# ortk95/planetmapper

Hardware: NVIDIA B200
Metric: full-backplane Mpix/s (FP64) + mapped-cube voxels/s at 1-8 B200 vs host CPU (higher is better)
Workload: dtype f64

## Files before the change

planetmapper_b200/csrc/backplane_kernels.cu:

```cuda
#include "pm_device.cuh"
#include "pm_kernels.h"

#include <cstdlib>

namespace pm {

constexpr int kPerThread = 4;
#ifndef PM_IMG_PARAM_CTAS
#define PM_IMG_PARAM_CTAS 4
#endif
constexpr int kImgParamCtas = PM_IMG_PARAM_CTAS;

__device__ __forceinline__ int slot(uint64_t mask, int k) { return __popcll(mask & (bit(k) - 1ull)); }

struct PlaneOffsets {
    int64_t byte_off[PM_N_PLANES];
    int64_t frame_stride;
};
static PlaneOffsets make_plane_offsets(uint64_t mask, int64_t plane_stride) {
    PlaneOffsets po;
    int slot = 0;
    for (int k = 0; k < PM_N_PLANES; k++) {
        po.byte_off[k] = (int64_t)slot * plane_stride * (int64_t)sizeof(double);
        if (mask & bit(k)) slot++;
    }
    po.frame_stride = (int64_t)slot * plane_stride;
    return po;
}

struct PlaneSink {
    char *base;
    const PlaneOffsets &po;
    __device__ __forceinline__ void put(int k, double v) const {
        __stcs(reinterpret_cast<double *>(base + po.byte_off[k]), v);
    }
};

template <bool kSky, uint64_t kFixedMask, bool kSpinSym>
__device__ __forceinline__ void img_tile(const FrameD &fs, uint32_t tile, uint32_t nx, uint32_t npx, int per_thread,
                                         uint64_t mask, const PlaneOffsets &po, double *__restrict__ out) {
    uint32_t idx = tile * (uint32_t)(kBlock * per_thread) + threadIdx.x;
    uint32_t yi = idx / nx, xi = idx - yi * nx;
#pragma unroll 1
    for (int r = 0; r < per_thread && idx < npx; r++) {
        PlaneSink sink{reinterpret_cast<char *>(out + idx), po};
        image_pixel<kSky, kFixedMask, false, kSpinSym>(fs, (double)xi, (double)yi, mask, sink);
        idx += kBlock;
        xi += kBlock;
        while (xi >= nx) {
            xi -= nx;
            yi++;
        }
    }
}

template <bool kSky, uint64_t kFixedMask>
__global__ void __launch_bounds__(kBlock, 4) backplanes_img_kernel(const PMFrame *__restrict__ frames, uint32_t nx,
                                                                   uint32_t npx, int per_thread, uint64_t mask,
                                                                   const __grid_constant__ PlaneOffsets po,
                                                                   double *__restrict__ out_all) {
    __shared__ FrameD fs;
    load_frame(fs, frames + blockIdx.y);
    double *out = out_all + (int64_t)blockIdx.y * __popcll(mask) * npx;
    if (fs.spin_sym)
        img_tile<kSky, kFixedMask, true>(fs, blockIdx.x, nx, npx, per_thread, mask, po, out);
    else
        img_tile<kSky, kFixedMask, false>(fs, blockIdx.x, nx, npx, per_thread, mask, po, out);
}

__device__ __forceinline__ uint32_t centre_out_tile(uint32_t k, uint32_t n_tiles, uint32_t centre) {
    const uint32_t lo = centre, hi = n_tiles - 1u - centre;
    const uint32_t j = (k + 1u) >> 1;
    if (j <= min(lo, hi)) return (k & 1u) ? centre + j : centre - j;
    return lo < hi ? k : n_tiles - 1u - k;
}
template <bool kSky, uint64_t kFixedMask, bool kSpinSym>
__global__ void __launch_bounds__(kBlock, kImgParamCtas) backplanes_img_param_kernel(
    const __grid_constant__ FrameD fs, uint32_t nx, uint32_t npx, int per_thread, uint32_t centre_tile, uint64_t mask,
    const __grid_constant__ PlaneOffsets po, double *__restrict__ out) {
    img_tile<kSky, kFixedMask, kSpinSym>(fs, centre_out_tile(blockIdx.x, gridDim.x, centre_tile), nx, npx, per_thread,
                                         mask, po, out);
}

template <bool kSky, bool kRingAll, bool kSpinSym>
__global__ void __launch_bounds__(kBlock, 4) backplanes_points_param_kernel(const __grid_constant__ FrameD fs,
                                                                            const double *__restrict__ x_in,
                                                                            const double *__restrict__ y_in,
                                                                            int64_t n, uint64_t mask,
                                                                            const __grid_constant__ PlaneOffsets po,
                                                                            double *__restrict__ out) {
    const int64_t first = (int64_t)blockIdx.x * (kBlock * kPerThread) + threadIdx.x;
#pragma unroll 1
    for (int r = 0; r < kPerThread; r++) {
        const int64_t idx = first + r * kBlock;
        if (idx >= n) break;
        PlaneSink sink{reinterpret_cast<char *>(out + idx), po};
        image_point<kSky, kRingAll, kSpinSym>(fs, __ldg(x_in + idx), __ldg(y_in + idx), mask, sink);
    }
}

constexpr uint64_t kXYMapMask = bit(PM_PIXEL_X) | bit(PM_PIXEL_Y);

template <uint64_t kFixedMask>
__device__ __forceinline__ void map_tile(const FrameD &fs, const double *__restrict__ lon_in,
                                         const double *__restrict__ lat_in, int64_t n, uint64_t mask,
                                         const PlaneOffsets &po, double *__restrict__ out) {
    const int64_t first = (int64_t)blockIdx.x * (kBlock * kPerThread) + threadIdx.x;
#pragma unroll 1
    for (int r = 0; r < kPerThread; r++) {
        const int64_t idx = first + r * kBlock;
        if (idx >= n) break;
        PlaneSink sink{reinterpret_cast<char *>(out + idx), po};
        map_cell<kFixedMask>(fs, __ldg(lon_in + idx), __ldg(lat_in + idx), mask, sink);
    }
// ... 198 lines not shown
                                  int64_t n, double *__restrict__ out) {
    const int64_t i = (int64_t)blockIdx.x * blockDim.x + threadIdx.x;
    if (i >= n) return;
    const double x = a[i], y = b ? b[i] : 0.0;
    double s, c, r = NAN;
    switch (kind) {
        case 0: r = fast_rcp(x); break;
        case 1: r = fast_rsqrt(x); break;
        case 2: r = fast_sqrt(x); break;
        case 3: sincos_small(x, s, c); r = s; break;
        case 4: sincos_small(x, s, c); r = c; break;
        case 5: r = fast_atan2(x, y); break;
        case 6: r = fast_acos(x); break;
        case 7: r = fast_div(x, y); break;
        case 8: sincos_full(x, s, c); r = s; break;
        case 9: sincos_full(x, s, c); r = c; break;
        case 10: r = fast_atan2_ypos(fabs(x), y); break;
        case 11: r = fast_atan2_xpos(x, fabs(y)); break;
        case 12: sincos_small2(x, 0.0, s, c, r, r); r = s; break;
        case 13: sincos_small2(x, 0.0, s, c, r, r); r = c; break;
        default: break;
    }
    out[i] = r;
}

static unsigned chunks_for(int64_t n) {
    const int64_t per = (int64_t)kBlock * kPerThread;
    int64_t blocks = (n + per - 1) / per;
    return (unsigned)(blocks < 1 ? 1 : blocks);
}

constexpr uint64_t kDefaultStackMask = kLonLatMask | kCentricMask | kIllumMask | kStateMask;

static int pick_per_thread(int64_t n, int64_t n_batches, int sm_count, int ctas_per_sm) {
    const int64_t tiles = ((n + kBlock - 1) / kBlock) * n_batches;
    const int64_t target = (int64_t)sm_count * ctas_per_sm * 3;
    int per = 16;
    while (per > 1 && tiles / per < target) per >>= 1;
    return per;
}

cudaError_t launch_backplanes_img(const PMFrame *frames, int n_frames, int nx, int ny, uint64_t mask,
                                  double *out, int sm_count, cudaStream_t st) {
    const int64_t npx = (int64_t)nx * ny;
    if (npx >= (1ll << 31)) return cudaErrorInvalidValue;
    const PlaneOffsets po = make_plane_offsets(mask, npx);
    static const int forced = tune_int("PM_IMG_PER_THREAD", 0);
    const int per = forced > 0 ? forced : pick_per_thread(npx, n_frames, sm_count, 4);
    const int64_t chunk = (int64_t)kBlock * per;
    dim3 grid((unsigned)((npx + chunk - 1) / chunk), n_frames);
    static const bool no_fixed = tune_int("PM_IMG_NO_FIXED_MASK", 0) != 0;
    if (mask == kDefaultStackMask && !no_fixed)
        backplanes_img_kernel<false, kDefaultStackMask><<<grid, kBlock, 0, st>>>(frames, (uint32_t)nx, (uint32_t)npx,
                                                                                   per, mask, po, out);
    else if (mask & kSkyMask)
        backplanes_img_kernel<true, 0><<<grid, kBlock, 0, st>>>(frames, (uint32_t)nx, (uint32_t)npx, per, mask, po, out);
    else
        backplanes_img_kernel<false, 0><<<grid, kBlock, 0, st>>>(frames, (uint32_t)nx, (uint32_t)npx, per, mask, po, out);
    count_launches(1);
    return cudaGetLastError();
}
template <bool kSpinSym>
static void launch_img_param(const FrameD &fs, dim3 grid, uint32_t nx, uint32_t npx, int per, uint32_t centre,
                             uint64_t mask, const PlaneOffsets &po, double *out, cudaStream_t st) {
    if (mask == kDefaultStackMask)
        backplanes_img_param_kernel<false, kDefaultStackMask, kSpinSym><<<grid, kBlock, 0, st>>>(fs, nx, npx, per, centre,
                                                                                                mask, po, out);
    else if (mask & kSkyMask)
        backplanes_img_param_kernel<true, 0, kSpinSym><<<grid, kBlock, 0, st>>>(fs, nx, npx, per, centre, mask, po, out);
    else
        backplanes_img_param_kernel<false, 0, kSpinSym><<<grid, kBlock, 0, st>>>(fs, nx, npx, per, centre, mask, po, out);
}
cudaError_t launch_backplanes_img_host(const PMFrame *frame_host, int nx, int ny, uint64_t mask, double *out,
                                       int sm_count, cudaStream_t st) {
    const int64_t npx = (int64_t)nx * ny;
    if (npx >= (1ll << 31)) return cudaErrorInvalidValue;
    FrameD fs;
    load_frame_host(fs, frame_host);
    const PlaneOffsets po = make_plane_offsets(mask, npx);
    static const int forced = tune_int("PM_IMG_PER_THREAD", 0);
    const int per = forced > 0 ? forced : pick_per_thread(npx, 1, sm_count, kImgParamCtas);
    const int64_t chunk = (int64_t)kBlock * per;
    const int64_t n_tiles = (npx + chunk - 1) / chunk;
    dim3 grid((unsigned)n_tiles, 1);
    double cy = frame_host->y0 < 0.0 ? 0.0 : (frame_host->y0 > ny - 1.0 ? ny - 1.0 : frame_host->y0);
    double cx = frame_host->x0 < 0.0 ? 0.0 : (frame_host->x0 > nx - 1.0 ? nx - 1.0 : frame_host->x0);
    if (!(cy == cy) || !(cx == cx)) cy = cx = 0.0;
    int64_t ct = ((int64_t)cy * nx + (int64_t)cx) / chunk;
    static const bool linear = tune_int("PM_IMG_ORDER", 1) == 0;
    if (linear) ct = 0;
    const uint32_t centre = (uint32_t)(ct < 0 ? 0 : (ct >= n_tiles ? n_tiles - 1 : ct));
    if (fs.spin_sym)
        launch_img_param<true>(fs, grid, (uint32_t)nx, (uint32_t)npx, per, centre, mask, po, out, st);
    else
        launch_img_param<false>(fs, grid, (uint32_t)nx, (uint32_t)npx, per, centre, mask, po, out, st);
    count_launches(1);
    return cudaGetLastError();
}
template <bool kSpinSym>
static void launch_points_param(const FrameD &fs, unsigned grid, const double *x, const double *y, int64_t n,
                                uint64_t mask, uint32_t flags, const PlaneOffsets &po, double *out, cudaStream_t st) {
    if (!(mask & kSkyMask))
        backplanes_points_param_kernel<false, false, kSpinSym><<<grid, kBlock, 0, st>>>(fs, x, y, n, mask, po, out);
    else if (flags & PM_FLAG_RING_ALL)
        backplanes_points_param_kernel<true, true, kSpinSym><<<grid, kBlock, 0, st>>>(fs, x, y, n, mask, po, out);
    else
        backplanes_points_param_kernel<true, false, kSpinSym><<<grid, kBlock, 0, st>>>(fs, x, y, n, mask, po, out);
}
cudaError_t launch_backplanes_points_host(const PMFrame *frame_host, const double *x, const double *y, int64_t n,
                                          uint64_t mask, uint32_t flags, double *out, cudaStream_t st) {
    FrameD fs;
    load_frame_host(fs, frame_host);
    const PlaneOffsets po = make_plane_offsets(mask, n);
    const unsigned grid = chunks_for(n);
    if (fs.spin_sym)
        launch_points_param<true>(fs, grid, x, y, n, mask, flags, po, out, st);
    else
        launch_points_param<false>(fs, grid, x, y, n, mask, flags, po, out, st);
    count_launches(1);
    return cudaGetLastError();
}
cudaError_t launch_backplanes_map(const PMFrame *frames, int n_frames, const double *lon, const double *lat,
                                  int64_t n, uint64_t mask, double *out, int sm_count, cudaStream_t st) {
    (void)sm_count;
    const dim3 grid(chunks_for(n), (unsigned)n_frames);
    const PlaneOffsets po = make_plane_offsets(mask, n);
    if (mask == kXYMapMask)
        backplanes_map_kernel<kXYMapMask><<<grid, kBlock, 0, st>>>(frames, lon, lat, n, mask, po, out);
// ... 87 lines not shown
```

planetmapper_b200/csrc/pm_device.cuh:

```cuda
#pragma once

#include "../../include/pm_b200.h"
#include "pm_math.cuh"

namespace pm {

struct V3 {
    double x, y, z;
};

PM_HD V3 mk(double x, double y, double z) { return V3{x, y, z}; }
PM_HD V3 operator+(V3 a, V3 b) { return mk(a.x + b.x, a.y + b.y, a.z + b.z); }
PM_HD V3 operator-(V3 a, V3 b) { return mk(a.x - b.x, a.y - b.y, a.z - b.z); }
PM_HD V3 operator-(V3 a) { return mk(-a.x, -a.y, -a.z); }
PM_HD V3 operator*(double s, V3 a) { return mk(s * a.x, s * a.y, s * a.z); }
PM_HD double dot(V3 a, V3 b) { return fma(a.x, b.x, fma(a.y, b.y, a.z * b.z)); }
PM_HD V3 cross(V3 a, V3 b) {
    return mk(fma(a.y, b.z, -a.z * b.y), fma(a.z, b.x, -a.x * b.z), fma(a.x, b.y, -a.y * b.x));
}
PM_HD V3 mul3(V3 a, const double *s) { return mk(a.x * s[0], a.y * s[1], a.z * s[2]); }
PM_HD V3 axpy(double s, V3 b, V3 a) { return mk(fma(s, b.x, a.x), fma(s, b.y, a.y), fma(s, b.z, a.z)); }
PM_HD double norm(V3 a) { return fast_sqrt_lite(dot(a, a)); }
PM_HD V3 ld3(const double *p) { return mk(p[0], p[1], p[2]); }
PM_HD bool finite3(V3 a) { return fabs(a.x) < INFINITY && fabs(a.y) < INFINITY && fabs(a.z) < INFINITY; }
PM_HD V3 mxv(const double *m, V3 v) {
    return mk(fma(m[0], v.x, fma(m[1], v.y, m[2] * v.z)), fma(m[3], v.x, fma(m[4], v.y, m[5] * v.z)),
              fma(m[6], v.x, fma(m[7], v.y, m[8] * v.z)));
}
PM_HD V3 mtxv(const double *m, V3 v) {
    return mk(fma(m[0], v.x, fma(m[3], v.y, m[6] * v.z)), fma(m[1], v.x, fma(m[4], v.y, m[7] * v.z)),
              fma(m[2], v.x, fma(m[5], v.y, m[8] * v.z)));
}
PM_HD_NOINLINE double pymod360_slow(double a) {
    double r = ::fmod(a, 360.0);
    if (r != 0.0 && r < 0.0) r += 360.0;
    return r;
}
PM_HD double pymod360(double a) { return (a >= 0.0 && a < 360.0) ? a : pymod360_slow(a); }

struct FrameD {
    PMFrame f;
    double inv_c;
    double inv_r[3];
    double nw[3];
    double k[3];
    double wn;
    double rp;
    double e2, ep2;
    double inv_omf2;
    double omf;
    double P0b[3], VTb[3], ATb[3], VOb[3], S0b[3], VSb[3];
    double G[9];
    double y0[3];
    double y0m2;
    double As[6];
    double inv_kmpa;
    int biaxial;
    int spin_sym;
};

constexpr int kDeriveItems = 13;

PM_HD double ex_mul(double a, double b) {
#ifdef __CUDA_ARCH__
    return __dmul_rn(a, b);
#else
    return a * b;
#endif
}
PM_HD double ex_add(double a, double b) {
#ifdef __CUDA_ARCH__
    return __dadd_rn(a, b);
#else
    return a + b;
#endif
}
PM_HD double ex_div(double a, double b) {
#ifdef __CUDA_ARCH__
    return __ddiv_rn(a, b);
#else
    return a / b;
#endif
}
PM_HD double ex_sqrt(double a) {
#ifdef __CUDA_ARCH__
    return __dsqrt_rn(a);
#else
    return ::sqrt(a);
#endif
}
PM_HD double ex_dot3(double a0, double b0, double a1, double b1, double a2, double b2) {
    return ex_add(ex_add(ex_mul(a0, b0), ex_mul(a1, b1)), ex_mul(a2, b2));
}

PM_HD void derive_frame_item(FrameD &s, int item) {
    const PMFrame &f = s.f;
    if (item >= 3 && item <= 8) {
        const double *src = item == 3 ? f.P0 : item == 4 ? f.VT : item == 5 ? f.AT : item == 6 ? f.VO : item == 7 ? f.S0 : f.VS;
        double *dst = item == 3 ? s.P0b : item == 4 ? s.VTb : item == 5 ? s.ATb : item == 6 ? s.VOb : item == 7 ? s.S0b : s.VSb;
        for (int r = 0; r < 3; r++)
            dst[r] = ex_dot3(f.R0[3 * r], src[0], f.R0[3 * r + 1], src[1], f.R0[3 * r + 2], src[2]);
        if (item == 3) {
            for (int r = 0; r < 3; r++) s.y0[r] = ex_mul(-dst[r], ex_div(1.0, f.radii[r]));
            s.y0m2 = fma(s.y0[0], s.y0[0], fma(s.y0[1], s.y0[1], ex_mul(s.y0[2], s.y0[2])));
        }
    } else if (item >= 9 && item <= 11) {
        const int r = item - 9;
        for (int c = 0; c < 3; c++)
            s.G[3 * r + c] = ex_dot3(f.R0[3 * r], f.M[3 * c], f.R0[3 * r + 1], f.M[3 * c + 1], f.R0[3 * r + 2], f.M[3 * c + 2]);
    } else if (item == 12) {
        const double sc = kRpd / 3600.0;
        for (int c = 0; c < 3; c++) {
            s.As[c] = -ex_mul(f.A[c], sc);
            s.As[3 + c] = ex_mul(f.A[3 + c], sc);
        }
        s.inv_kmpa = ex_div(1.0, f.km_per_arcsec);
    } else if (item == 0) {
        s.inv_c = ex_div(1.0, f.clight);
        const double w2 = ex_dot3(f.omega[0], f.omega[0], f.omega[1], f.omega[1], f.omega[2], f.omega[2]);
        const double wn = ex_sqrt(w2);
        s.wn = wn;
        s.k[0] = wn > 0.0 ? ex_div(f.omega[0], wn) : 0.0;
        s.k[1] = wn > 0.0 ? ex_div(f.omega[1], wn) : 0.0;
        s.k[2] = wn > 0.0 ? ex_div(f.omega[2], wn) : 0.0;
        const double wperp = ex_sqrt(ex_add(ex_mul(f.omega[0], f.omega[0]), ex_mul(f.omega[1], f.omega[1])));
        const double flat = fabs(ex_add(f.radii[0], -f.radii[2]));
        const double shift = ex_mul(ex_mul(wperp, ex_div(ex_mul(2.0, f.radii[0]), f.clight)), flat);
        s.spin_sym = (f.radii[0] == f.radii[1]) && (shift <= 1.0e-9);
    } else if (item == 1) {
        const double a = f.radii[0], b = f.radii[1], c = f.radii[2];
        s.inv_r[0] = ex_div(1.0, a);
        s.inv_r[1] = ex_div(1.0, b);
        s.inv_r[2] = ex_div(1.0, c);
        const double m = fmin(a, fmin(b, c));
        const double ma = ex_div(m, a), mb = ex_div(m, b), mc = ex_div(m, c);
        s.nw[0] = ex_mul(ma, ma);
        s.nw[1] = ex_mul(mb, mb);
        s.nw[2] = ex_mul(mc, mc);
    } else if (item == 2) {
        const double rp = ex_add(f.re, -ex_mul(f.f, f.re));
        const double re2 = ex_mul(f.re, f.re), rp2 = ex_mul(rp, rp);
        const double omf = ex_add(1.0, -f.f);
        s.rp = rp;
        s.e2 = ex_add(1.0, -ex_div(rp2, re2));
        s.ep2 = ex_add(ex_div(re2, rp2), -1.0);
        s.omf = omf;
        s.inv_omf2 = ex_div(1.0, ex_mul(omf, omf));
        s.biaxial = (f.radii[0] == f.radii[1]) && (f.re == f.radii[0]) && (fabs(rp - f.radii[2]) <= 4e-16 * f.radii[2]);
    }
}

#ifdef __CUDACC__
__device__ __forceinline__ void load_frame(FrameD &s, const PMFrame *__restrict__ g) {
    const double *src = reinterpret_cast<const double *>(g);
    double *dst = reinterpret_cast<double *>(&s.f);
    for (int i = threadIdx.x; i < PM_FRAME_NDOUBLES; i += blockDim.x) dst[i] = __ldg(src + i);
    __syncthreads();
    const int w = threadIdx.x >> 5, l = threadIdx.x & 31;
    int item = -1;
    if (blockDim.x >= 128) {
        if (w == 0 && l < 6) item = 3 + l;
// ... 57 lines not shown
    const double ku = dot(k, u);
    const V3 t = mk(fma(k.x, ku, -u.x), fma(k.y, ku, -u.y), fma(k.z, ku, -u.z));
    return axpy(r.omc, t, axpy(r.s, kxu, u));
}
PM_HD V3 spin_bwd(const FrameD &fs, Rot r, V3 u) { return spin_bwd_c(fs, r, u, cross(ld3(fs.k), u)); }
PM_HD V3 to_body(const FrameD &fs, Rot r, V3 v) { return spin_fwd(fs, r, mxv(fs.f.R0, v)); }
PM_HD V3 from_body(const FrameD &fs, Rot r, V3 u) { return mtxv(fs.f.R0, spin_bwd(fs, r, u)); }
PM_HD V3 target_pos_b(const FrameD &fs, double dt) {
    const double h = 0.5 * dt * dt;
    return mk(fma(fs.ATb[0], h, fma(fs.VTb[0], dt, fs.P0b[0])), fma(fs.ATb[1], h, fma(fs.VTb[1], dt, fs.P0b[1])),
              fma(fs.ATb[2], h, fma(fs.VTb[2], dt, fs.P0b[2])));
}

PM_HD void recrad_angles(V3 v, double &ra, double &dec) {
    dec = fast_atan2_xpos(v.z, fast_sqrt(fma(v.x, v.x, v.y * v.y)));
    double lon = fast_atan2(v.y, v.x);
    if (lon < 0.0) lon += kTwoPi;
    ra = lon;
}
PM_HD V3 radrec1(double ra, double dec) {
    double sr, cr, sd, cd;
    sincos_full(ra, sr, cr);
    sincos_full(dec, sd, cd);
    return mk(cr * cd, sr * cd, sd);
}
PM_HD double vsep(V3 a, V3 b) { return fast_atan2_ypos(norm(cross(a, b)), dot(a, b)); }

struct RayHit {
    V3 pp;
    double ixx;
    double a;
    double t;
    double cos2;
};
PM_HD bool surfpt_yx(const FrameD &fs, V3 y, double ym2, V3 x, double ixx, V3 &p, RayHit &hit) {
    const double yx = dot(y, x);
    const double a = -(yx * ixx);
    const V3 pp = axpy(a, x, y);
    const double pm2 = dot(pp, pp);
    if (!(pm2 < INFINITY)) return false;
    hit.pp = pp;
    hit.ixx = ixx;
    hit.a = a;
    hit.cos2 = 1.0 - pm2;
    double h;
    if (ym2 > 1.0) {
        if (pm2 > 1.0) return false;
        if (yx > 0.0) return false;
        h = -fast_sqrt_lite((1.0 - pm2) * ixx);
    } else if (ym2 == 1.0) {
        h = -a;
    } else {
        h = fast_sqrt_lite(fmax(0.0, 1.0 - pm2) * ixx);
    }
    hit.t = a + h;
    p = mul3(axpy(h, x, pp), fs.f.radii);
    return true;
}
PM_HD bool surfpt_y(const FrameD &fs, V3 y, double ym2, V3 u, V3 &p, RayHit &hit) {
    const V3 x = mul3(u, fs.inv_r);
    const double xx = dot(x, x);
    if (!(xx > 0.0)) return false;
    return surfpt_yx(fs, y, ym2, x, fast_rcp(xx), p, hit);
}
PM_HD bool surfpt(const FrameD &fs, V3 o, V3 u, V3 &p, RayHit &hit) {
    const V3 y = mul3(o, fs.inv_r);
    return surfpt_y(fs, y, dot(y, y), u, p, hit);
}

struct Intercept {
    V3 p;
    V3 u;
    V3 p0;
    Rot r;
    double dt;
    double L;
    double lt;
};

template <bool kSpinSym>
PM_HD_NOINLINE bool sincpt_converge(const FrameD &fs, V3 u0, double &dt, V3 &p, double &range) {
    const PMFrame &f = fs.f;
    for (int it = 0; it < 8; it++) {
        V3 o = -target_pos_b(fs, dt), u = u0;
        if (!kSpinSym) {
            const Rot r = make_rot(fs, dt);
            o = spin_fwd(fs, r, o);
            u = spin_fwd(fs, r, u0);
        }
        RayHit hit;
        if (!surfpt(fs, o, u, p, hit)) return false;
        range = hit.t;
        const double t = dt + f.t_ref;
        const double t_new = f.et - hit.t * fs.inv_c;
        if (!(fabs(t_new - t) > 1.0e-17 * fabs(t_new))) break;
        dt = t_new - f.t_ref;
    }
    return true;
}

template <bool kSpinSym = false>
PM_HD bool sincpt(const FrameD &fs, V3 u0, Intercept &it) {
    const PMFrame &f = fs.f;
    V3 p1, p2;
    RayHit h1, h2;
    const V3 x = mul3(u0, fs.inv_r);
    const double xx = dot(x, x);
    if (!(xx > 0.0)) return false;
    const double ixx = fast_rcp(xx);
    if (!surfpt_yx(fs, ld3(fs.y0), fs.y0m2, x, ixx, p1, h1)) return false;
    const double lt1 = h1.t * fs.inv_c;

    const double dt1 = (f.et - lt1) - f.t_ref;
    if (kSpinSym) {
        const V3 y2 = mul3(-target_pos_b(fs, dt1), fs.inv_r);
        if (!surfpt_yx(fs, y2, dot(y2, y2), x, ixx, p2, h2)) return false;
    } else {
        const Rot r1 = make_rot(fs, dt1);
        if (!surfpt(fs, spin_fwd(fs, r1, -target_pos_b(fs, dt1)), spin_fwd(fs, r1, u0), p2, h2)) return false;
    }
    const double lt2 = h2.t * fs.inv_c;

    double dt = (f.et - lt2) - f.t_ref;
    V3 p;
    double L;
    if (fabs(dt1) > PM_T(kPixC)[kPixDt1Min] && h2.cos2 > PM_T(kPixC)[kPixGrazing]) {
        const double lam = fast_div_lite(dt - dt1, dt1 - (dt - dt1));
        dt = fma(lam, dt1, dt1) + f.t_ref;
        dt -= f.t_ref;
        const V3 pps = axpy(lam, h2.pp - h1.pp, h2.pp);
        const double ixxs = kSpinSym ? ixx : fma(lam, h2.ixx - h1.ixx, h2.ixx);
        const double hs = fast_sqrt_lite(fmax(1.0 - dot(pps, pps), 0.0) * ixxs);
        L = fma(lam, h2.a - h1.a, h2.a) - hs;
        it.r = make_rot(fs, dt);
        if (kSpinSym) {
            it.p0 = axpy(-hs, u0, mul3(pps, fs.f.radii));
            p = spin_fwd(fs, it.r, it.p0);
        } else {
            it.u = spin_fwd(fs, it.r, u0);
            p = axpy(-hs, it.u, mul3(pps, fs.f.radii));
        }
    } else {
        double dt_c = dt, L_c;
        V3 p_c;
        if (!sincpt_converge<kSpinSym>(fs, u0, dt_c, p_c, L_c)) return false;
        dt = dt_c;
        L = L_c;
        it.r = make_rot(fs, dt);
        if (kSpinSym) {
            it.p0 = p_c;
            p = spin_fwd(fs, it.r, p_c);
        } else {
            p = p_c;
            it.u = spin_fwd(fs, it.r, u0);
        }
    }
    it.p = p;
    it.dt = dt;
    it.L = L;
    it.lt = L * fs.inv_c;
    return true;
}

PM_HD void geodetic_general(const FrameD &fs, double rho, double z, double &lat, double &alt) {
    const PMFrame &f = fs.f;
    if (f.f == 0.0) {
        lat = fast_atan2_xpos(z, rho);
        alt = fast_sqrt(fma(rho, rho, z * z)) - f.re;
        return;
    }
    double sb = f.re * z, cb = fs.rp * rho;
    double n = fast_rsqrt(fma(sb, sb, cb * cb) + sqrt_guard());
    sb *= n;
    cb *= n;
    double num = z, den = rho;
// ... 152 lines not shown
#pragma unroll 1
    for (int pass = 0; pass < 2; pass++) {
        const double dt = (f.et - lt) - f.t_ref;
        const Rot r = make_rot(fs, dt);
        const V3 p0 = spin_bwd(fs, r, p);
        const V3 X0 = target_pos_b(fs, dt) + p0;
        const double L = norm(X0);
        lt = L * fs.inv_c;
        g.p0 = p0;
        g.X0 = X0;
        g.r = r;
        g.dt = dt;
        g.L = L;
        g.lt = lt;
    }
}
PM_HD double point_rv(const FrameD &fs, V3 p, const PointGeom &g) {
    const double iL = fast_rcp(g.L);
    const V3 ph0 = iL * g.X0;
    const V3 vt = axpy(g.dt, ld3(fs.ATb), ld3(fs.VTb));
    const V3 vrot0 = spin_bwd(fs, g.r, cross(ld3(fs.f.omega), p));
    const double a = dot(vt + vrot0, ph0);
    const double b = dot(ld3(fs.VOb), ph0);
    return radial_velocity(fs, a, b);
}

PM_HD V3 xy2ray_local(const FrameD &fs, double x, double y) {
    const double ra = fma(fs.As[0], x, fma(fs.As[1], y, fs.As[2]));
    const double dec = fma(fs.As[3], x, fma(fs.As[4], y, fs.As[5]));
    double sr, cr, sd, cd;
    sincos_small2(ra, dec, sr, cr, sd, cd);
    return mk(cr * cd, sr * cd, sd);
}

PM_HD void obsvec2angular(const PMFrame &f, V3 ov, double &ax, double &ay) {
    double ra, dec;
    recrad_angles(mxv(f.M, ov), ra, dec);
    double x = pymod360(-(ra * kDpr));
    if (x > 180.0) x -= 360.0;
    ax = x * 3600.0;
    ay = (dec * kDpr) * 3600.0;
}

PM_HD V3 targvec2obsvec(const FrameD &fs, V3 tv) {
    const PMFrame &f = fs.f;
    const V3 off = tv - ld3(f.sub_t);
    const double dist_offset = norm(ld3(f.sub_ray) + off) - f.sub_dist;
    const double sub_et = f.t_ref + f.sub_dt;
    const double tt = sub_et - dist_offset * fs.inv_c;
    const Rot r = make_rot(fs, tt - f.t_ref);
    return ld3(f.sub_obs) + from_body(fs, r, off);
}

PM_HD V3 obsvec2targvec(const FrameD &fs, V3 ov) {
    const PMFrame &f = fs.f;
    const V3 off = ov - ld3(f.sub_obs);
    const double dist_offset = norm(off - ld3(f.sub_ray)) - f.sub_dist;
    const double sub_et = f.t_ref + f.sub_dt;
    const double tt = sub_et - dist_offset * fs.inv_c;
    const Rot r = make_rot(fs, tt - f.t_ref);
    return ld3(f.sub_t) + to_body(fs, r, off);
}

PM_HD void ring_coordinates(const FrameD &fs, V3 ov, double &radius, double &lon_deg, double &dist) {
    const PMFrame &f = fs.f;
    radius = lon_deg = dist = NAN;
// ... 12 lines not shown

PM_HD void limb_coordinates(const FrameD &fs, V3 ov, double &lon_deg, double &lat_deg, double &dist) {
    const PMFrame &f = fs.f;
    lon_deg = lat_deg = dist = NAN;
    const double n2 = dot(ov, ov);
    if (!(n2 > 0.0)) return;
    const V3 u = fast_rsqrt(n2) * ov;
    const V3 P0 = ld3(f.P0);
    const V3 pn = dot(P0, u) * u;
    const double near_dist = norm(P0 - pn);
    const V3 tv = obsvec2targvec(fs, pn);
    const V3 x = mul3(tv, fs.inv_r);
    const double xn2 = dot(x, x);
    if (!(xn2 > 0.0)) return;
    const V3 sp = fast_rsqrt(xn2) * tv;
    double lon, lat, alt;
    recpgr(fs, sp, fs.biaxial != 0, lon, lat, alt);
    lon_deg = lon * kDpr;
    lat_deg = lat * kDpr;
    dist = near_dist - norm(sp);
}

PM_HD constexpr uint64_t bit(int k) { return 1ull << k; }
constexpr uint64_t kKmMask = bit(PM_KM_X) | bit(PM_KM_Y) | bit(PM_ANGULAR_X) | bit(PM_ANGULAR_Y);
constexpr uint64_t kLonLatMask = bit(PM_LON_GRAPHIC) | bit(PM_LAT_GRAPHIC) | bit(PM_LOCAL_SOLAR_TIME);
constexpr uint64_t kCentricMask = bit(PM_LON_CENTRIC) | bit(PM_LAT_CENTRIC);
constexpr uint64_t kIllumMask = bit(PM_PHASE) | bit(PM_INCIDENCE) | bit(PM_EMISSION) | bit(PM_AZIMUTH);
constexpr uint64_t kStateMask = bit(PM_DISTANCE) | bit(PM_RADIAL_VELOCITY) | bit(PM_DOPPLER);
constexpr uint64_t kLimbMask = bit(PM_LIMB_DISTANCE) | bit(PM_LIMB_LON_GRAPHIC) | bit(PM_LIMB_LAT_GRAPHIC);
constexpr uint64_t kRingMask = bit(PM_RING_RADIUS) | bit(PM_RING_LON_GRAPHIC) | bit(PM_RING_DISTANCE);
constexpr uint64_t kSurfMask = kLonLatMask | kCentricMask | kIllumMask | kStateMask | kRingMask;
constexpr uint64_t kSkyMask = bit(PM_RA) | bit(PM_DEC) | kKmMask | kLimbMask | kRingMask;

template <bool kSky, uint64_t kFixedMask = 0, bool kRingAll = false, bool kSpinSym = false, class Sink>
PM_HD void image_pixel(const FrameD &fs, double x, double y, uint64_t mask_in, Sink &out) {
    const PMFrame &f = fs.f;
    const double nan = NAN;
    const uint64_t mask = kFixedMask ? kFixedMask : (kSky ? mask_in : (mask_in & ~kSkyMask));
    if (mask & bit(PM_PIXEL_X)) out.put(PM_PIXEL_X, x);
    if (mask & bit(PM_PIXEL_Y)) out.put(PM_PIXEL_Y, y);

    const double dx = x - f.x0, dy = y - f.y0;
    const bool try_disc = (mask & kSurfMask) && !(f.optimize_speed != 0.0 && fma(dx, dx, dy * dy) > f.r_cut2);
    V3 v = mk(nan, nan, nan);
    if (try_disc || (kSky && (mask & kSkyMask))) v = xy2ray_local(fs, x, y);
    V3 d2 = mk(nan, nan, nan);
    if (kSky && (mask & kSkyMask)) {
        const V3 d = mtxv(f.M, v);
        double ra, dec;
        recrad_angles(d, ra, dec);
        const double ra_deg = ra * kDpr, dec_deg = dec * kDpr;
        if (mask & bit(PM_RA)) out.put(PM_RA, ra_deg);
        if (mask & bit(PM_DEC)) out.put(PM_DEC, dec_deg);
        if (mask & (kKmMask | kLimbMask | kRingMask)) d2 = radrec1(ra_deg * kRpd, dec_deg * kRpd);
        if (mask & kKmMask) {
            double ax, ay;
            obsvec2angular(f, d2, ax, ay);
            const double kx = fma(f.ang2km[0], ax, f.ang2km[1] * ay);
            const double ky = fma(f.ang2km[2], ax, f.ang2km[3] * ay);
            if (mask & bit(PM_KM_X)) out.put(PM_KM_X, kx);
            if (mask & bit(PM_KM_Y)) out.put(PM_KM_Y, ky);
            if (mask & bit(PM_ANGULAR_X)) out.put(PM_ANGULAR_X, fast_div(kx, f.km_per_arcsec));
            if (mask & bit(PM_ANGULAR_Y)) out.put(PM_ANGULAR_Y, fast_div(ky, f.km_per_arcsec));
        }
    }

    bool on_disc = false;
    Intercept it;
    const V3 u0 = mxv(fs.G, v);
    if (try_disc) on_disc = sincpt<kSpinSym>(fs, u0, it);

    double v_dist = nan;
    if (on_disc) {
        const V3 p = it.p;
        if (mask & (kLonLatMask | kCentricMask)) {
            const double rho = fast_sqrt_lite(fma(p.x, p.x, p.y * p.y));
            const double lon_e = fast_atan2(p.y, p.x);
            if (mask & kLonLatMask) {
// ... 31 lines not shown
            if (mask & bit(PM_DISTANCE)) out.put(PM_DISTANCE, v_dist);
            if (mask & (bit(PM_RADIAL_VELOCITY) | bit(PM_DOPPLER))) {
                const V3 vt = axpy(it.dt, ld3(fs.ATb), ld3(fs.VTb));
                const double a = fma(fs.wn, dot(kxp, kSpinSym ? u0 : it.u), dot(vt, u0));
                const double b = dot(ld3(fs.VOb), u0);
                const double rv = radial_velocity(fs, a, b);
                if (mask & bit(PM_RADIAL_VELOCITY)) out.put(PM_RADIAL_VELOCITY, rv);
                if (mask & bit(PM_DOPPLER)) out.put(PM_DOPPLER, doppler_factor(fs, rv));
            }
        }
    } else {
        const uint64_t m = mask & (kLonLatMask | kCentricMask | kIllumMask | kStateMask);
#pragma unroll
        for (int k = 0; k <= PM_DOPPLER; k++)
            if ((kLonLatMask | kCentricMask | kIllumMask | kStateMask) & bit(k))
                if (m & bit(k)) out.put(k, nan);
    }

    if (kSky && (mask & kLimbMask)) {
        double llon, llat, ldist;
        limb_coordinates(fs, d2, llon, llat, ldist);
        if (mask & bit(PM_LIMB_DISTANCE)) out.put(PM_LIMB_DISTANCE, ldist);
        if (mask & bit(PM_LIMB_LON_GRAPHIC)) out.put(PM_LIMB_LON_GRAPHIC, llon);
        if (mask & bit(PM_LIMB_LAT_GRAPHIC)) out.put(PM_LIMB_LAT_GRAPHIC, llat);
    }
    if (kSky && (mask & kRingMask)) {
        double rad, rl, rd;
        ring_coordinates(fs, d2, rad, rl, rd);
        if (!kRingAll && rd > v_dist) rad = rl = rd = nan;
        if (mask & bit(PM_RING_RADIUS)) out.put(PM_RING_RADIUS, rad);
        if (mask & bit(PM_RING_LON_GRAPHIC)) out.put(PM_RING_LON_GRAPHIC, rl);
        if (mask & bit(PM_RING_DISTANCE)) out.put(PM_RING_DISTANCE, rd);
    }
}

template <bool kSky, bool kRingAll, bool kSpinSym = false, class Sink>
PM_HD void image_point(const FrameD &fs, double x, double y, uint64_t mask_in, Sink &out) {
    if (fabs(x) < INFINITY && fabs(y) < INFINITY) {
        image_pixel<kSky, 0, kRingAll, kSpinSym>(fs, x, y, mask_in, out);
        return;
    }
#pragma unroll 1
    for (int k = 0; k < PM_N_PLANES; k++)
        if (mask_in & bit(k)) out.put(k, k == PM_PIXEL_X ? x : (k == PM_PIXEL_Y ? y : (double)NAN));
}

template <uint64_t kFixedMask = 0, class Sink>
PM_HD void map_cell(const FrameD &fs, double lon_deg, double lat_deg, uint64_t mask_in, Sink &out) {
    const uint64_t mask = kFixedMask ? kFixedMask : mask_in;
    const PMFrame &f = fs.f;
    const double nan = NAN;
    const double lonm = (fabs(lon_deg) < INFINITY) ? pymod360(lon_deg) : nan;
    const double latm = (fabs(lat_deg) < INFINITY) ? lat_deg : nan;
    if (mask & bit(PM_LON_GRAPHIC)) out.put(PM_LON_GRAPHIC, lonm);
    if (mask & bit(PM_LAT_GRAPHIC)) out.put(PM_LAT_GRAPHIC, latm);
    const bool lon_ok = lonm == lonm;
    const bool ok = lon_ok && (latm == latm);
    if (mask & bit(PM_LOCAL_SOLAR_TIME))
        out.put(PM_LOCAL_SOLAR_TIME, lon_ok ? local_solar_time(f, lonm) : nan);

    double v_clon = nan, v_clat = nan, v_g = nan, v_i = nan, v_e = nan, v_az = nan, v_dist = nan, v_rv = nan,
           v_dop = nan, v_ra = nan, v_dec = nan, v_x = nan, v_y = nan, v_kx = nan, v_ky = nan, v_ax = nan,
           v_ay = nan;
    double limb_lon = nan, limb_lat = nan, limb_dist = nan, ring_rad = nan, ring_lon = nan, ring_dist = nan;
    if (ok) {
        const V3 tv = pgrrec0(fs, lonm * kRpd, latm * kRpd);
// ... 252 lines not shown
```

Before: 32780.

## Tile image into 2D blocks with separable ray sincos and perturbative spin-symmetric second hit

Switches the image backplane kernels from linear per-thread chunks to 2D tiles (one column per thread, several rows per block). When the pixel-to-sky affine map is axis-aligned and small, per-row and per-column sin/cos are computed once and shared through shared memory. For spin-symmetric targets, the second light-time surface intercept is replaced by a first-order perturbation of the first hit using a cached reciprocal sqrt. The spin-symmetric path is also narrowed with an observer-outside check. This cuts redundant trig and surface-intersection work, but adds a __syncthreads per block and approximation risk in the separable ray and perturbative intercept.

```diff
diff --git a/planetmapper_b200/csrc/backplane_kernels.cu b/planetmapper_b200/csrc/backplane_kernels.cu
--- a/planetmapper_b200/csrc/backplane_kernels.cu
+++ b/planetmapper_b200/csrc/backplane_kernels.cu
@@ -36,50 +36,73 @@
     }
 };
 
+constexpr int kMaxTileRows = 16;
+
+struct TileRay {
+    const FrameD &fs;
+    double x, y, sr, cr;
+    const double2 *row;
+    __device__ __forceinline__ V3 operator()() const {
+        if (!fs.ray_sep) return xy2ray_local(fs, x, y);
+        const double2 d = *row;
+        return mk(cr * d.y, sr * d.y, d.x);
+    }
+};
+
 template <bool kSky, uint64_t kFixedMask, bool kSpinSym>
-__device__ __forceinline__ void img_tile(const FrameD &fs, uint32_t tile, uint32_t nx, uint32_t npx, int per_thread,
-                                         uint64_t mask, const PlaneOffsets &po, double *__restrict__ out) {
-    uint32_t idx = tile * (uint32_t)(kBlock * per_thread) + threadIdx.x;
-    uint32_t yi = idx / nx, xi = idx - yi * nx;
-#pragma unroll 1
-    for (int r = 0; r < per_thread && idx < npx; r++) {
-        PlaneSink sink{reinterpret_cast<char *>(out + idx), po};
-        image_pixel<kSky, kFixedMask, false, kSpinSym>(fs, (double)xi, (double)yi, mask, sink);
-        idx += kBlock;
-        xi += kBlock;
-        while (xi >= nx) {
-            xi -= nx;
-            yi++;
-        }
+__device__ __forceinline__ void img_tile(const FrameD &fs, uint32_t tx, uint32_t ty, uint32_t nx, uint32_t ny,
+                                         int rows, uint64_t mask, const PlaneOffsets &po, double *__restrict__ out) {
+    __shared__ double2 row_sc[kMaxTileRows];
+    const uint32_t xi = tx * kBlock + threadIdx.x, y_first = ty * (uint32_t)rows;
+    if (fs.ray_sep && threadIdx.x < rows) {
+        double sd, cd;
+        ray_row(fs, (double)(y_first + threadIdx.x), sd, cd);
+        row_sc[threadIdx.x] = make_double2(sd, cd);
+    }
+    __syncthreads();
+    if (xi >= nx) return;
+    const double x = (double)xi;
+    double sr = 0.0, cr = 0.0;
+    if (fs.ray_sep) ray_col(fs, x, sr, cr);
+    const int n_rows = (int)min((uint32_t)rows, ny - y_first);
+#pragma unroll 1
+    for (int r = 0; r < n_rows; r++) {
+        const uint32_t yi = y_first + (uint32_t)r;
+        PlaneSink sink{reinterpret_cast<char *>(out + (yi * nx + xi)), po};
+        image_pixel_ray<kSky, kFixedMask, false, kSpinSym>(fs, x, (double)yi, mask, sink,
+                                                           TileRay{fs, x, (double)yi, sr, cr, row_sc + r});
     }
 }
 
 template <bool kSky, uint64_t kFixedMask>
 __global__ void __launch_bounds__(kBlock, 4) backplanes_img_kernel(const PMFrame *__restrict__ frames, uint32_t nx,
-                                                                   uint32_t npx, int per_thread, uint64_t mask,
+                                                                   uint32_t ny, uint32_t n_tx, int rows, uint64_t mask,
                                                                    const __grid_constant__ PlaneOffsets po,
                                                                    double *__restrict__ out_all) {
     __shared__ FrameD fs;
     load_frame(fs, frames + blockIdx.y);
-    double *out = out_all + (int64_t)blockIdx.y * __popcll(mask) * npx;
+    double *out = out_all + (int64_t)blockIdx.y * __popcll(mask) * nx * ny;
+    const uint32_t ty = blockIdx.x / n_tx, tx = blockIdx.x - ty * n_tx;
     if (fs.spin_sym)
-        img_tile<kSky, kFixedMask, true>(fs, blockIdx.x, nx, npx, per_thread, mask, po, out);
-    else
-        img_tile<kSky, kFixedMask, false>(fs, blockIdx.x, nx, npx, per_thread, mask, po, out);
-}
-
-__device__ __forceinline__ uint32_t centre_out_tile(uint32_t k, uint32_t n_tiles, uint32_t centre) {
-    const uint32_t lo = centre, hi = n_tiles - 1u - centre;
+        img_tile<kSky, kFixedMask, true>(fs, tx, ty, nx, ny, rows, mask, po, out);
+    else
+        img_tile<kSky, kFixedMask, false>(fs, tx, ty, nx, ny, rows, mask, po, out);
+}
+
+__device__ __forceinline__ uint32_t centre_out(uint32_t k, uint32_t n, uint32_t centre) {
+    const uint32_t lo = centre, hi = n - 1u - centre;
     const uint32_t j = (k + 1u) >> 1;
     if (j <= min(lo, hi)) return (k & 1u) ? centre + j : centre - j;
-    return lo < hi ? k : n_tiles - 1u - k;
+    return lo < hi ? k : n - 1u - k;
 }
 template <bool kSky, uint64_t kFixedMask, bool kSpinSym>
 __global__ void __launch_bounds__(kBlock, kImgParamCtas) backplanes_img_param_kernel(
-    const __grid_constant__ FrameD fs, uint32_t nx, uint32_t npx, int per_thread, uint32_t centre_tile, uint64_t mask,
-    const __grid_constant__ PlaneOffsets po, double *__restrict__ out) {
-    img_tile<kSky, kFixedMask, kSpinSym>(fs, centre_out_tile(blockIdx.x, gridDim.x, centre_tile), nx, npx, per_thread,
-                                         mask, po, out);
+    const __grid_constant__ FrameD fs, uint32_t nx, uint32_t ny, uint32_t n_tx, int rows, uint32_t centre_tx,
+    uint32_t centre_ty, uint64_t mask, const __grid_constant__ PlaneOffsets po, double *__restrict__ out) {
+    const uint32_t n_ty = gridDim.x / n_tx;
+    const uint32_t ky = blockIdx.x / n_tx, kx = blockIdx.x - ky * n_tx;
+    img_tile<kSky, kFixedMask, kSpinSym>(fs, centre_out(kx, n_tx, centre_tx), centre_out(ky, n_ty, centre_ty), nx, ny,
+                                         rows, mask, po, out);
 }
 
 template <bool kSky, bool kRingAll, bool kSpinSym>
@@ -344,12 +367,14 @@
 
 constexpr uint64_t kDefaultStackMask = kLonLatMask | kCentricMask | kIllumMask | kStateMask;
 
-static int pick_per_thread(int64_t n, int64_t n_batches, int sm_count, int ctas_per_sm) {
-    const int64_t tiles = ((n + kBlock - 1) / kBlock) * n_batches;
+static int pick_rows(int nx, int ny, int64_t n_batches, int sm_count, int ctas_per_sm) {
+    static const int forced = tune_int("PM_IMG_PER_THREAD", 0);
+    if (forced > 0) return forced < kMaxTileRows ? forced : kMaxTileRows;
+    const int64_t n_tx = (nx + kBlock - 1) / kBlock;
     const int64_t target = (int64_t)sm_count * ctas_per_sm * 3;
-    int per = 16;
-    while (per > 1 && tiles / per < target) per >>= 1;
-    return per;
+    int rows = kMaxTileRows;
+    while (rows > 1 && n_tx * ((ny + rows - 1) / rows) * n_batches < target) rows >>= 1;
+    return rows;
 }
 
 cudaError_t launch_backplanes_img(const PMFrame *frames, int n_frames, int nx, int ny, uint64_t mask,
@@ -357,31 +382,40 @@
     const int64_t npx = (int64_t)nx * ny;
     if (npx >= (1ll << 31)) return cudaErrorInvalidValue;
     const PlaneOffsets po = make_plane_offsets(mask, npx);
-    static const int forced = tune_int("PM_IMG_PER_THREAD", 0);
-    const int per = forced > 0 ? forced : pick_per_thread(npx, n_frames, sm_count, 4);
-    const int64_t chunk = (int64_t)kBlock * per;
-    dim3 grid((unsigned)((npx + chunk - 1) / chunk), n_frames);
+    const int rows = pick_rows(nx, ny, n_frames, sm_count, 4);
+    const uint32_t n_tx = (uint32_t)((nx + kBlock - 1) / kBlock), n_ty = (uint32_t)((ny + rows - 1) / rows);
+    dim3 grid(n_tx * n_ty, n_frames);
     static const bool no_fixed = tune_int("PM_IMG_NO_FIXED_MASK", 0) != 0;
     if (mask == kDefaultStackMask && !no_fixed)
-        backplanes_img_kernel<false, kDefaultStackMask><<<grid, kBlock, 0, st>>>(frames, (uint32_t)nx, (uint32_t)npx,
-                                                                                   per, mask, po, out);
+        backplanes_img_kernel<false, kDefaultStackMask><<<grid, kBlock, 0, st>>>(frames, (uint32_t)nx, (uint32_t)ny,
+                                                                                   n_tx, rows, mask, po, out);
     else if (mask & kSkyMask)
-        backplanes_img_kernel<true, 0><<<grid, kBlock, 0, st>>>(frames, (uint32_t)nx, (uint32_t)npx, per, mask, po, out);
-    else
-        backplanes_img_kernel<false, 0><<<grid, kBlock, 0, st>>>(frames, (uint32_t)nx, (uint32_t)npx, per, mask, po, out);
+        backplanes_img_kernel<true, 0><<<grid, kBlock, 0, st>>>(frames, (uint32_t)nx, (uint32_t)ny, n_tx, rows, mask,
+                                                                po, out);
+    else
+        backplanes_img_kernel<false, 0><<<grid, kBlock, 0, st>>>(frames, (uint32_t)nx, (uint32_t)ny, n_tx, rows, mask,
+                                                                 po, out);
     count_launches(1);
     return cudaGetLastError();
 }
 template <bool kSpinSym>
-static void launch_img_param(const FrameD &fs, dim3 grid, uint32_t nx, uint32_t npx, int per, uint32_t centre,
-                             uint64_t mask, const PlaneOffsets &po, double *out, cudaStream_t st) {
+static void launch_img_param(const FrameD &fs, dim3 grid, uint32_t nx, uint32_t ny, uint32_t n_tx, int rows,
+                             uint32_t ctx, uint32_t cty, uint64_t mask, const PlaneOffsets &po, double *out,
+                             cudaStream_t st) {
     if (mask == kDefaultStackMask)
-        backplanes_img_param_kernel<false, kDefaultStackMask, kSpinSym><<<grid, kBlock, 0, st>>>(fs, nx, npx, per, centre,
-                                                                                                mask, po, out);
+        backplanes_img_param_kernel<false, kDefaultStackMask, kSpinSym><<<grid, kBlock, 0, st>>>(
+            fs, nx, ny, n_tx, rows, ctx, cty, mask, po, out);
     else if (mask & kSkyMask)
-        backplanes_img_param_kernel<true, 0, kSpinSym><<<grid, kBlock, 0, st>>>(fs, nx, npx, per, centre, mask, po, out);
-    else
-        backplanes_img_param_kernel<false, 0, kSpinSym><<<grid, kBlock, 0, st>>>(fs, nx, npx, per, centre, mask, po, out);
+        backplanes_img_param_kernel<true, 0, kSpinSym><<<grid, kBlock, 0, st>>>(fs, nx, ny, n_tx, rows, ctx, cty, mask,
+                                                                                po, out);
+    else
+        backplanes_img_param_kernel<false, 0, kSpinSym><<<grid, kBlock, 0, st>>>(fs, nx, ny, n_tx, rows, ctx, cty,
+                                                                                 mask, po, out);
+}
+static uint32_t centre_tile(double c, int n, int tile) {
+    if (!(c == c)) return 0;
+    c = c < 0.0 ? 0.0 : (c > n - 1.0 ? n - 1.0 : c);
+    return (uint32_t)((int64_t)c / tile);
 }
 cudaError_t launch_backplanes_img_host(const PMFrame *frame_host, int nx, int ny, uint64_t mask, double *out,
                                        int sm_count, cudaStream_t st) {
@@ -390,22 +424,16 @@
     FrameD fs;
     load_frame_host(fs, frame_host);
     const PlaneOffsets po = make_plane_offsets(mask, npx);
-    static const int forced = tune_int("PM_IMG_PER_THREAD", 0);
-    const int per = forced > 0 ? forced : pick_per_thread(npx, 1, sm_count, kImgParamCtas);
-    const int64_t chunk = (int64_t)kBlock * per;
-    const int64_t n_tiles = (npx + chunk - 1) / chunk;
-    dim3 grid((unsigned)n_tiles, 1);
-    double cy = frame_host->y0 < 0.0 ? 0.0 : (frame_host->y0 > ny - 1.0 ? ny - 1.0 : frame_host->y0);
-    double cx = frame_host->x0 < 0.0 ? 0.0 : (frame_host->x0 > nx - 1.0 ? nx - 1.0 : frame_host->x0);
-    if (!(cy == cy) || !(cx == cx)) cy = cx = 0.0;
-    int64_t ct = ((int64_t)cy * nx + (int64_t)cx) / chunk;
+    const int rows = pick_rows(nx, ny, 1, sm_count, kImgParamCtas);
+    const uint32_t n_tx = (uint32_t)((nx + kBlock - 1) / kBlock), n_ty = (uint32_t)((ny + rows - 1) / rows);
+    dim3 grid(n_tx * n_ty, 1);
     static const bool linear = tune_int("PM_IMG_ORDER", 1) == 0;
-    if (linear) ct = 0;
-    const uint32_t centre = (uint32_t)(ct < 0 ? 0 : (ct >= n_tiles ? n_tiles - 1 : ct));
+    const uint32_t ctx = linear ? 0 : centre_tile(frame_host->x0, nx, kBlock);
+    const uint32_t cty = linear ? 0 : centre_tile(frame_host->y0, ny, rows);
     if (fs.spin_sym)
-        launch_img_param<true>(fs, grid, (uint32_t)nx, (uint32_t)npx, per, centre, mask, po, out, st);
-    else
-        launch_img_param<false>(fs, grid, (uint32_t)nx, (uint32_t)npx, per, centre, mask, po, out, st);
+        launch_img_param<true>(fs, grid, (uint32_t)nx, (uint32_t)ny, n_tx, rows, ctx, cty, mask, po, out, st);
+    else
+        launch_img_param<false>(fs, grid, (uint32_t)nx, (uint32_t)ny, n_tx, rows, ctx, cty, mask, po, out, st);
     count_launches(1);
     return cudaGetLastError();
 }
diff --git a/planetmapper_b200/csrc/pm_device.cuh b/planetmapper_b200/csrc/pm_device.cuh
--- a/planetmapper_b200/csrc/pm_device.cuh
+++ b/planetmapper_b200/csrc/pm_device.cuh
@@ -54,9 +54,11 @@
     double y0[3];
     double y0m2;
     double As[6];
+    double Vs[3], Ws[3];
     double inv_kmpa;
     int biaxial;
     int spin_sym;
+    int ray_sep;
 };
 
 constexpr int kDeriveItems = 13;
@@ -100,9 +102,10 @@
         double *dst = item == 3 ? s.P0b : item == 4 ? s.VTb : item == 5 ? s.ATb : item == 6 ? s.VOb : item == 7 ? s.S0b : s.VSb;
         for (int r = 0; r < 3; r++)
             dst[r] = ex_dot3(f.R0[3 * r], src[0], f.R0[3 * r + 1], src[1], f.R0[3 * r + 2], src[2]);
-        if (item == 3) {
-            for (int r = 0; r < 3; r++) s.y0[r] = ex_mul(-dst[r], ex_div(1.0, f.radii[r]));
-            s.y0m2 = fma(s.y0[0], s.y0[0], fma(s.y0[1], s.y0[1], ex_mul(s.y0[2], s.y0[2])));
+        if (item <= 5) {
+            double *w = item == 3 ? s.y0 : item == 4 ? s.Vs : s.Ws;
+            for (int r = 0; r < 3; r++) w[r] = ex_mul(-dst[r], ex_div(1.0, f.radii[r]));
+            if (item == 3) s.y0m2 = fma(s.y0[0], s.y0[0], fma(s.y0[1], s.y0[1], ex_mul(s.y0[2], s.y0[2])));
         }
     } else if (item >= 9 && item <= 11) {
         const int r = item - 9;
@@ -115,6 +118,19 @@
             s.As[3 + c] = ex_mul(f.A[3 + c], sc);
         }
         s.inv_kmpa = ex_div(1.0, f.km_per_arcsec);
+        s.ray_sep = 0;
+        if (s.As[1] == 0.0 && s.As[3] == 0.0) {
+            const double ra0 = fma(s.As[0], 0.0, fma(s.As[1], 0.0, s.As[2]));
+            const double ra1 = fma(s.As[0], f.nx - 1.0, fma(s.As[1], 0.0, s.As[2]));
+            const double de0 = fma(s.As[3], 0.0, fma(s.As[4], 0.0, s.As[5]));
+            const double de1 = fma(s.As[3], 0.0, fma(s.As[4], f.ny - 1.0, s.As[5]));
+            const double hi = fmax(fmax(fabs(ra0), fabs(ra1)), fmax(fabs(de0), fabs(de1)));
+            const double t = 0.00390625;
+            const bool far = (ra0 > t && ra1 > t) || (ra0 < -t && ra1 < -t) || (de0 > t && de1 > t) ||
+                             (de0 < -t && de1 < -t);
+            if (hi <= t) s.ray_sep = 1;
+            else if (hi <= PM_T(kMisc)[1] && far) s.ray_sep = 2;
+        }
     } else if (item == 0) {
         s.inv_c = ex_div(1.0, f.clight);
         const double w2 = ex_dot3(f.omega[0], f.omega[0], f.omega[1], f.omega[1], f.omega[2], f.omega[2]);
@@ -126,7 +142,15 @@
         const double wperp = ex_sqrt(ex_add(ex_mul(f.omega[0], f.omega[0]), ex_mul(f.omega[1], f.omega[1])));
         const double flat = fabs(ex_add(f.radii[0], -f.radii[2]));
         const double shift = ex_mul(ex_mul(wperp, ex_div(ex_mul(2.0, f.radii[0]), f.clight)), flat);
-        s.spin_sym = (f.radii[0] == f.radii[1]) && (shift <= 1.0e-9);
+        const double rmax = fmax(f.radii[0], fmax(f.radii[1], f.radii[2]));
+        const double rmin = fmin(f.radii[0], fmin(f.radii[1], f.radii[2]));
+        const double dtm = ex_mul(ex_mul(2.0, rmax), s.inv_c);
+        const double vn = ex_add(ex_add(fabs(f.VT[0]), fabs(f.VT[1])), fabs(f.VT[2]));
+        const double an = ex_add(ex_add(fabs(f.AT[0]), fabs(f.AT[1])), fabs(f.AT[2]));
+        const double pn = fmax(fabs(f.P0[0]), fmax(fabs(f.P0[1]), fabs(f.P0[2])));
+        const double move = ex_mul(dtm, ex_add(vn, ex_mul(ex_mul(0.5, dtm), an)));
+        const bool outside = ex_mul(ex_add(pn, -rmax), rmin) > ex_mul(ex_mul(2.0, move), rmax);
+        s.spin_sym = (f.radii[0] == f.radii[1]) && (shift <= 1.0e-9) && outside;
     } else if (item == 1) {
         const double a = f.radii[0], b = f.radii[1], c = f.radii[2];
         s.inv_r[0] = ex_div(1.0, a);
@@ -250,6 +274,7 @@
     double a;
     double t;
     double cos2;
+    double ih;
 };
 PM_HD bool surfpt_yx(const FrameD &fs, V3 y, double ym2, V3 x, double ixx, V3 &p, RayHit &hit) {
     const double yx = dot(y, x);
@@ -265,7 +290,9 @@
     if (ym2 > 1.0) {
         if (pm2 > 1.0) return false;
         if (yx > 0.0) return false;
-        h = -fast_sqrt_lite((1.0 - pm2) * ixx);
+        const double hh = (1.0 - pm2) * ixx;
+        hit.ih = fast_rsqrt(hh + sqrt_guard());
+        h = -(hh * hit.ih);
     } else if (ym2 == 1.0) {
         h = -a;
     } else {
@@ -330,26 +357,41 @@
     const double lt1 = h1.t * fs.inv_c;
 
     const double dt1 = (f.et - lt1) - f.t_ref;
+    V3 dpp;
+    double da;
+    double cos2;
+    double lt2;
     if (kSpinSym) {
-        const V3 y2 = mul3(-target_pos_b(fs, dt1), fs.inv_r);
-        if (!surfpt_yx(fs, y2, dot(y2, y2), x, ixx, p2, h2)) return false;
+        const double hd = 0.5 * dt1;
+        const V3 delta = dt1 * mk(fma(hd, fs.Ws[0], fs.Vs[0]), fma(hd, fs.Ws[1], fs.Vs[1]), fma(hd, fs.Ws[2], fs.Vs[2]));
+        da = -(dot(delta, x) * ixx);
+        dpp = axpy(da, x, delta);
+        const double D = dot(axpy(2.0, h1.pp, dpp), dpp);
+        cos2 = h1.cos2 - D;
+        if (!(cos2 >= 0.0) || h1.a + da < 0.0) return false;
+        const double k = 0.5 * h1.ih;
+        const double dH0 = -(D * ixx) * k;
+        const double dH = fma(-(dH0 * k), dH0, dH0);
+        lt2 = (h1.t + (da - dH)) * fs.inv_c;
     } else {
         const Rot r1 = make_rot(fs, dt1);
         if (!surfpt(fs, spin_fwd(fs, r1, -target_pos_b(fs, dt1)), spin_fwd(fs, r1, u0), p2, h2)) return false;
-    }
-    const double lt2 = h2.t * fs.inv_c;
+        cos2 = h2.cos2;
+        lt2 = h2.t * fs.inv_c;
+    }
 
     double dt = (f.et - lt2) - f.t_ref;
     V3 p;
     double L;
-    if (fabs(dt1) > PM_T(kPixC)[kPixDt1Min] && h2.cos2 > PM_T(kPixC)[kPixGrazing]) {
+    if (fabs(dt1) > PM_T(kPixC)[kPixDt1Min] && cos2 > PM_T(kPixC)[kPixGrazing]) {
         const double lam = fast_div_lite(dt - dt1, dt1 - (dt - dt1));
         dt = fma(lam, dt1, dt1) + f.t_ref;
         dt -= f.t_ref;
-        const V3 pps = axpy(lam, h2.pp - h1.pp, h2.pp);
+        const double lp1 = 1.0 + lam;
+        const V3 pps = kSpinSym ? axpy(lp1, dpp, h1.pp) : axpy(lam, h2.pp - h1.pp, h2.pp);
         const double ixxs = kSpinSym ? ixx : fma(lam, h2.ixx - h1.ixx, h2.ixx);
         const double hs = fast_sqrt_lite(fmax(1.0 - dot(pps, pps), 0.0) * ixxs);
-        L = fma(lam, h2.a - h1.a, h2.a) - hs;
+        L = (kSpinSym ? fma(lp1, da, h1.a) : fma(lam, h2.a - h1.a, h2.a)) - hs;
         it.r = make_rot(fs, dt);
         if (kSpinSym) {
             it.p0 = axpy(-hs, u0, mul3(pps, fs.f.radii));
@@ -359,6 +401,7 @@
             p = axpy(-hs, it.u, mul3(pps, fs.f.radii));
         }
     } else {
+        if (kSpinSym) dt = (f.et - ((h1.a + da) - fast_sqrt_lite(cos2 * ixx)) * fs.inv_c) - f.t_ref;
         double dt_c = dt, L_c;
         V3 p_c;
         if (!sincpt_converge<kSpinSym>(fs, u0, dt_c, p_c, L_c)) return false;
@@ -577,6 +620,18 @@
     sincos_small2(ra, dec, sr, cr, sd, cd);
     return mk(cr * cd, sr * cd, sd);
 }
+PM_HD void sincos_tier(int tier, double a, double &s, double &c) {
+    if (tier == 1)
+        sincos_tiny(a, s, c);
+    else
+        sincos_quarter(a, s, c);
+}
+PM_HD void ray_col(const FrameD &fs, double x, double &sr, double &cr) {
+    sincos_tier(fs.ray_sep, fma(fs.As[0], x, fma(fs.As[1], 0.0, fs.As[2])), sr, cr);
+}
+PM_HD void ray_row(const FrameD &fs, double y, double &sd, double &cd) {
+    sincos_tier(fs.ray_sep, fma(fs.As[3], 0.0, fma(fs.As[4], y, fs.As[5])), sd, cd);
+}
 
 PM_HD void obsvec2angular(const PMFrame &f, V3 ov, double &ax, double &ay) {
     double ra, dec;
@@ -655,8 +710,8 @@
 constexpr uint64_t kSurfMask = kLonLatMask | kCentricMask | kIllumMask | kStateMask | kRingMask;
 constexpr uint64_t kSkyMask = bit(PM_RA) | bit(PM_DEC) | kKmMask | kLimbMask | kRingMask;
 
-template <bool kSky, uint64_t kFixedMask = 0, bool kRingAll = false, bool kSpinSym = false, class Sink>
-PM_HD void image_pixel(const FrameD &fs, double x, double y, uint64_t mask_in, Sink &out) {
+template <bool kSky, uint64_t kFixedMask = 0, bool kRingAll = false, bool kSpinSym = false, class Sink, class RayFn>
+PM_HD void image_pixel_ray(const FrameD &fs, double x, double y, uint64_t mask_in, Sink &out, const RayFn &ray) {
     const PMFrame &f = fs.f;
     const double nan = NAN;
     const uint64_t mask = kFixedMask ? kFixedMask : (kSky ? mask_in : (mask_in & ~kSkyMask));
@@ -666,7 +721,7 @@
     const double dx = x - f.x0, dy = y - f.y0;
     const bool try_disc = (mask & kSurfMask) && !(f.optimize_speed != 0.0 && fma(dx, dx, dy * dy) > f.r_cut2);
     V3 v = mk(nan, nan, nan);
-    if (try_disc || (kSky && (mask & kSkyMask))) v = xy2ray_local(fs, x, y);
+    if (try_disc || (kSky && (mask & kSkyMask))) v = ray();
     V3 d2 = mk(nan, nan, nan);
     if (kSky && (mask & kSkyMask)) {
         const V3 d = mtxv(f.M, v);
@@ -764,6 +819,16 @@
         if (mask & bit(PM_RING_LON_GRAPHIC)) out.put(PM_RING_LON_GRAPHIC, rl);
         if (mask & bit(PM_RING_DISTANCE)) out.put(PM_RING_DISTANCE, rd);
     }
+}
+
+struct PixelRay {
+    const FrameD &fs;
+    double x, y;
+    PM_HD V3 operator()() const { return xy2ray_local(fs, x, y); }
+};
+template <bool kSky, uint64_t kFixedMask = 0, bool kRingAll = false, bool kSpinSym = false, class Sink>
+PM_HD void image_pixel(const FrameD &fs, double x, double y, uint64_t mask_in, Sink &out) {
+    image_pixel_ray<kSky, kFixedMask, kRingAll, kSpinSym>(fs, x, y, mask_in, out, PixelRay{fs, x, y});
 }
 
 template <bool kSky, bool kRingAll, bool kSpinSym = false, class Sink>
```

Result: slower. 30000, median of 6 (-8.5%).
